# culiver/VAR

Hardware: AMD Instinct MI355X
Metric: 256x256 images/sec (CFG=1.5) VAR-d16 (higher is better)
Workload: dtype f32

## Files before the change

var_amd/csrc/winograd.hip:

```cpp
#include <cstdlib>
#include <type_traits>

#include "common.h"

namespace {

constexpr int WG_PT = 18;
constexpr int WG_NDMA = 21;
constexpr int WG_STAGE = WG_NDMA * 16 * 64;
constexpr int WG_ZSTR = 20;
constexpr int WG_LDS = 2 * WG_STAGE;
static_assert(8 * 64 * WG_ZSTR * 4 <= WG_LDS, "epilogue exchange must fit in the K-loop stages");

struct WinoP {
    const float* in; const float* u; const float* bias; const float* resid; float* out; double* gn_part;
    int H, W, Cin, Cout, ncg, pw, ppi;
};

__device__ __forceinline__ void wg_wait_dma_barrier() { asm volatile("s_waitcnt vmcnt(8)\n\ts_barrier" ::: "memory"); }

constexpr int WG_KO_NOEPI = 1, WG_KO_NOGN = 2, WG_KO_NORES = 4, WG_KO_NOBTDB = 8;

__device__ __forceinline__ int wg_swz(int pix) { return (pix >> 1) & 3; }

template <bool RES, bool GN, int KO>
__global__ void __launch_bounds__(256, 2) k_conv3x3_wino(WinoP p) {
    extern __shared__ __attribute__((aligned(16))) float smem[];
    const int tid = threadIdx.x, lane = tid & 63, wave = __builtin_amdgcn_readfirstlane(tid >> 6);
    const int r16 = lane & 15, kq = lane >> 4;
    int lin;
    {
        const int nwg = gridDim.x, bid = blockIdx.x, q = nwg >> 3, rem = nwg & 7, xcd = bid & 7, loc = bid >> 3;
        lin = (xcd < rem ? xcd * (q + 1) : rem * (q + 1) + (xcd - rem) * q) + loc;
    }
    const int cg = lin % p.ncg, pidx = lin / p.ncg, b = pidx / p.ppi, pi = pidx - b * p.ppi, py = pi / p.pw, px = pi - py * p.pw;
    const int y0 = py * 16, x0 = px * 16, c0 = cg * 32;
    const int H = p.H, W = p.W, Cin = p.Cin, Cout = p.Cout, nk = Cin >> 4;

    const int64_t img = (int64_t)H * W * Cin;
    const __amdgpu_buffer_rsrc_t rsrc = __builtin_amdgcn_make_buffer_rsrc((void*)(p.in + (int64_t)b * img), 0, (int)(img * 4), 0x00020000);
    uint32_t doff[6];
#pragma unroll
    for (int i = 0; i < 6; ++i) {
        const int pix = (wave + 4 * i) * 16 + (lane >> 2), c = lane & 3;
        const int yy = y0 - 1 + pix / WG_PT, xx = x0 - 1 + pix % WG_PT;
        const bool ok = pix < WG_PT * WG_PT && (unsigned)yy < (unsigned)H && (unsigned)xx < (unsigned)W;
        doff[i] = ok ? (uint32_t)((((int64_t)yy * W + xx) * Cin + ((c ^ wg_swz(pix)) << 2)) * 4) : 0x80000000u;
    }
    const uint32_t lds0 = (uint32_t)(uintptr_t)(__attribute__((address_space(3))) void*)smem;
    auto dma = [&](int kt, int st) {
#pragma unroll
        for (int i = 0; i < 6; ++i)
            if (wave + 4 * i < WG_NDMA) vh_dma16_buf(rsrc, doff[i], (uint32_t)kt * 64u, lds0 + st * WG_STAGE + (wave + 4 * i) * 1024);
    };

    const uint32_t ustr_xi = (uint32_t)nk * Cout * 64, ustr_kt = (uint32_t)Cout * 64;
    const __amdgpu_buffer_rsrc_t ursrc = __builtin_amdgcn_make_buffer_rsrc((void*)p.u, 0, (int)(16 * ustr_xi), 0x00020000);
    const uint32_t uoff = (uint32_t)((c0 + r16) * 16 + 4 * kq) * 4u;
    f32x4 u[4][2];
    auto load_u = [&](int kt, int j) {
#pragma unroll
        for (int cb = 0; cb < 2; ++cb)
            u[j][cb] = __builtin_bit_cast(f32x4, __builtin_amdgcn_raw_buffer_load_b128(
                ursrc, uoff, __builtin_amdgcn_readfirstlane((uint32_t)(4 * wave + j) * ustr_xi + (uint32_t)kt * ustr_kt + cb * 1024u), 0));
    };
    dma(0, 0);
#pragma unroll
    for (int j = 0; j < 4; ++j) { load_u(0, j); __builtin_amdgcn_sched_barrier(0); }

    const int ra = wave == 3 ? 1 : (wave == 2 ? 2 : wave), rb = wave == 0 ? 2 : (wave == 1 ? 2 : (wave == 2 ? 1 : 3));
    const float sg = wave == 1 ? 1.0f : -1.0f;
    uint32_t roff[2][4];
#pragma unroll
    for (int c = 0; c < 4; ++c) {
        const int pa = (2 * (r16 >> 3) + ra) * WG_PT + 2 * (r16 & 7) + c, pb = (2 * (r16 >> 3) + rb) * WG_PT + 2 * (r16 & 7) + c;
        roff[0][c] = (uint32_t)(pa * 64 + ((kq ^ wg_swz(pa)) << 4));
        roff[1][c] = (uint32_t)(pb * 64 + ((kq ^ wg_swz(pb)) << 4));
    }

    f32x4 acc[4][4][2];
#pragma unroll
    for (int j = 0; j < 4; ++j)
#pragma unroll
        for (int tb = 0; tb < 4; ++tb)
#pragma unroll
            for (int cb = 0; cb < 2; ++cb) acc[j][tb][cb] = f32x4{0.f, 0.f, 0.f, 0.f};

    const int et = tid & 63, eq = tid >> 6;
    const int ety = et >> 3, etx = et & 7;
    const int64_t obase = (((int64_t)b * H + y0 + 2 * ety) * W + x0 + 2 * etx) * Cout + c0 + 4 * eq;
    f32x4 b4[2], rs[2][2][2];
    auto epi_load = [&](int j) {
        if constexpr (KO & WG_KO_NOEPI) return;
        if (j == 0) { b4[0] = *(const f32x4*)(p.bias + c0 + 4 * eq); b4[1] = *(const f32x4*)(p.bias + c0 + 16 + 4 * eq); }
        if constexpr (RES) {
#pragma unroll
            for (int bb = 0; bb < 2; ++bb) rs[j >> 1][j & 1][bb] = *(const f32x4*)(p.resid + obase + ((int64_t)(j & 1) * W + bb) * Cout + (j >> 1) * 16);
        }
    };

    auto compute = [&](int st, int kt_dma, int kt_u, auto last) {
        const char* sb = (const char*)smem + st * WG_STAGE;
#pragma unroll
        for (int tb = 0; tb < 4; ++tb) {
            f32x4 da[4], db[4];
#pragma unroll
            for (int c = 0; c < 4; ++c) {
                da[c] = *(const f32x4*)(sb + roff[0][c] + tb * 72 * 64);
                db[c] = *(const f32x4*)(sb + roff[1][c] + tb * 72 * 64);
            }
            float e[4][4];
            if constexpr (!(KO & WG_KO_NOBTDB)) {
#pragma unroll
                for (int c = 0; c < 4; ++c)
#pragma unroll
                    for (int s = 0; s < 4; ++s) e[c][s] = __builtin_fmaf(sg, db[c][s], da[c][s]);
            }
#pragma unroll
            for (int j = 0; j < 4; ++j) {
#pragma unroll
                for (int s = 0; s < 4; ++s) {
                    float v;
                    if constexpr (KO & WG_KO_NOBTDB) v = (j & 1) ? db[j][s] : da[j][s];
                    else v = j == 0 ? e[0][s] - e[2][s] : (j == 1 ? e[1][s] + e[2][s] : (j == 2 ? e[2][s] - e[1][s] : e[1][s] - e[3][s]));
#pragma unroll
                    for (int cb = 0; cb < 2; ++cb) acc[j][tb][cb] = __builtin_amdgcn_mfma_f32_16x16x4f32(u[j][cb][s], v, acc[j][tb][cb], 0, 0, 0);
                }
                if (tb == 3) {
                    __builtin_amdgcn_sched_barrier(0);
                    if constexpr (decltype(last)::value) epi_load(j); else load_u(kt_u, j);
                }
            }
            __builtin_amdgcn_sched_barrier(0);
            if (tb == 0 && !decltype(last)::value) dma(kt_dma, st ^ 1);
        }
    };

    wg_wait_dma_barrier();
    int kt = 0;
    for (; kt + 2 < nk; kt += 2) {
        compute(0, kt + 1, kt + 1, std::false_type{});
        wg_wait_dma_barrier();
        compute(1, kt + 2, kt + 2, std::false_type{});
        wg_wait_dma_barrier();
    }
    compute(0, kt + 1, kt + 1, std::false_type{});
    wg_wait_dma_barrier();
    compute(1, 0, 0, std::true_type{});
    __builtin_amdgcn_s_barrier();
    if constexpr (KO & WG_KO_NOEPI) {
#pragma unroll
        for (int j = 0; j < 4; ++j)
#pragma unroll
            for (int tb = 0; tb < 4; ++tb)
#pragma unroll
                for (int cb = 0; cb < 2; ++cb) asm volatile("" :: "v"(acc[j][tb][cb]));
        return;
    }

    float* zb = smem;
    const int nblk = (H * W) >> 7;
#pragma unroll
    for (int cb = 0; cb < 2; ++cb) {
#pragma unroll
        for (int tb = 0; tb < 4; ++tb) {
            const f32x4 m0 = acc[0][tb][cb], m1 = acc[1][tb][cb], m2 = acc[2][tb][cb], m3 = acc[3][tb][cb];
            const f32x4 z0 = (m0 + m1) + m2, z1 = (m1 - m2) - m3;
            const int t = tb * 16 + r16;
            *(f32x4*)(zb + ((wave * 2 + 0) * 64 + t) * WG_ZSTR + 4 * kq) = z0;
            *(f32x4*)(zb + ((wave * 2 + 1) * 64 + t) * WG_ZSTR + 4 * kq) = z1;
        }
        __syncthreads();
        f32x4 z[4][2];
#pragma unroll
        for (int i = 0; i < 4; ++i)
#pragma unroll
            for (int bb = 0; bb < 2; ++bb) z[i][bb] = *(const f32x4*)(zb + ((i * 2 + bb) * 64 + et) * WG_ZSTR + 4 * eq);
        const int co = c0 + cb * 16 + 4 * eq;
        double gs[4] = {0.0, 0.0, 0.0, 0.0}, gq[4] = {0.0, 0.0, 0.0, 0.0};
#pragma unroll
        for (int a = 0; a < 2; ++a)
#pragma unroll
            for (int bb = 0; bb < 2; ++bb) {
                const f32x4 yv = a == 0 ? (z[0][bb] + z[1][bb]) + z[2][bb] : (z[1][bb] - z[2][bb]) - z[3][bb];
                f32x4 v = yv + b4[cb];
                const int64_t o = obase + ((int64_t)a * W + bb) * Cout + cb * 16;
                if constexpr (RES) v = rs[cb][a][bb] + v;
                *(f32x4*)(p.out + o) = v;
                if constexpr (GN) {
#pragma unroll
                    for (int e = 0; e < 4; ++e) { const double d = (double)v[e]; gs[e] += d; gq[e] += d * d; }
                }
            }
        if constexpr (GN) {
            const double t8[8] = {gs[0], gq[0], gs[1], gq[1], gs[2], gq[2], gs[3], gq[3]};
            const bool h4 = lane & 16, h3 = lane & 8, h2 = lane & 4;
            double r4[4], r2[2], r1;
#pragma unroll
            for (int i = 0; i < 4; ++i) r4[i] = (h4 ? t8[4 + i] : t8[i]) + __shfl_xor(h4 ? t8[i] : t8[4 + i], 16, 64);
#pragma unroll
            for (int i = 0; i < 2; ++i) r2[i] = (h3 ? r4[2 + i] : r4[i]) + __shfl_xor(h3 ? r4[i] : r4[2 + i], 8, 64);
            r1 = (h2 ? r2[1] : r2[0]) + __shfl_xor(h2 ? r2[0] : r2[1], 4, 64);
            r1 += __shfl_xor(r1, 2, 64);
            r1 += __shfl_xor(r1, 1, 64);
            if ((lane & 3) == 0)
                p.gn_part[(((int64_t)b * nblk + 2 * pi + (lane >> 5)) * Cout + co) * 2 + ((lane >> 2) & 7)] = r1;
        }
        if (cb == 0) __syncthreads();
    }
}

constexpr int WU_PS = 12;
constexpr int WU_NDMA = 8;
constexpr int WU_STAGE = WU_NDMA * 16 * 64;
constexpr int WU_LDS = 2 * WU_STAGE;

__device__ __forceinline__ void wu_wait_dma_barrier() { asm volatile("s_waitcnt vmcnt(9)\n\ts_barrier" ::: "memory"); }

template <bool GN>
__global__ void __launch_bounds__(256, 2) k_conv3x3_wino_up(WinoP p) {
    extern __shared__ __attribute__((aligned(16))) float smem[];
    const int tid = threadIdx.x, lane = tid & 63, wave = __builtin_amdgcn_readfirstlane(tid >> 6);
    const int r16 = lane & 15, kq = lane >> 4, th = wave & 1, ch = wave >> 1;
    int lin;
    {
        const int nwg = gridDim.x, bid = blockIdx.x, q = nwg >> 3, rem = nwg & 7, xcd = bid & 7, loc = bid >> 3;
        lin = (xcd < rem ? xcd * (q + 1) : rem * (q + 1) + (xcd - rem) * q) + loc;
    }
    const int cg = lin % p.ncg, pidx = lin / p.ncg, b = pidx / p.ppi, pi = pidx - b * p.ppi, py = pi / p.pw, px = pi - py * p.pw;
    const int y0 = py * 16, x0 = px * 16, c0 = cg * 32 + ch * 16;
    const int H = p.H, W = p.W, Hi = H >> 1, Wi = W >> 1, Cin = p.Cin, Cout = p.Cout, nk = Cin >> 4;

    const int64_t img = (int64_t)Hi * Wi * Cin;
    const __amdgpu_buffer_rsrc_t rsrc = __builtin_amdgcn_make_buffer_rsrc((void*)(p.in + (int64_t)b * img), 0, (int)(img * 4), 0x00020000);
    uint32_t doff[2];
#pragma unroll
    for (int i = 0; i < 2; ++i) {
        const int pix = (wave + 4 * i) * 16 + (lane >> 2), c = lane & 3;
        const int pr = pix / WU_PS, pc = pix - pr * WU_PS;
        const int yy = (y0 >> 1) - 1 + pr, xx = (x0 >> 1) - 1 + pc;
        const bool ok = pr < 10 && pc < 10 && (unsigned)yy < (unsigned)Hi && (unsigned)xx < (unsigned)Wi;
        doff[i] = ok ? (uint32_t)((((int64_t)yy * Wi + xx) * Cin + ((c ^ ((pr & 1) << 1)) << 2)) * 4) : 0x80000000u;
    }
    const uint32_t lds0 = (uint32_t)(uintptr_t)(__attribute__((address_space(3))) void*)smem;
    auto dma = [&](int kt, int st) __attribute__((always_inline)) {
#pragma unroll
        for (int i = 0; i < 2; ++i) vh_dma16_buf(rsrc, doff[i], (uint32_t)kt * 64u, lds0 + st * WU_STAGE + (wave + 4 * i) * 1024);
    };

    const __amdgpu_buffer_rsrc_t ursrc = __builtin_amdgcn_make_buffer_rsrc((void*)p.u, 0, (int)(64u * Cin * Cout), 0x00020000);
    const uint32_t uoff = (uint32_t)((c0 + r16) * 4 * Cin + 4 * kq) * 4u;
    f32x4 u[9];
    auto load_u = [&](int kt, int r) __attribute__((always_inline)) {
#pragma unroll
        for (int c = 0; c < 3; ++c)
            u[3 * r + c] = __builtin_bit_cast(f32x4, __builtin_amdgcn_raw_buffer_load_b128(
                ursrc, uoff, __builtin_amdgcn_readfirstlane((uint32_t)((((r == 2 ? 2 : 0) + (c == 2 ? 1 : 0)) * Cout * 4 + (r == 0 ? 0 : 2) + (c == 0 ? 0 : 1)) * Cin + 16 * kt) * 4u), 0));
    };
    dma(0, 0);
#pragma unroll
    for (int r = 0; r < 3; ++r) { load_u(0, r); __builtin_amdgcn_sched_barrier(0); }

    const int prow = 4 * th + (r16 >> 3), pbase = (prow * WU_PS + (r16 & 7)) * 64;
    const uint32_t roff_e = (uint32_t)(pbase + ((kq ^ ((prow & 1) << 1)) << 4)), roff_o = (uint32_t)(pbase + ((kq ^ (((prow + 1) & 1) << 1)) << 4));

    f32x4 acc[9][2];
#pragma unroll
    for (int j = 0; j < 9; ++j)
#pragma unroll
        for (int tb = 0; tb < 2; ++tb) acc[j][tb] = f32x4{0.f, 0.f, 0.f, 0.f};

    f32x4 b4;
    auto compute = [&](int st, int kt_dma, int kt_u, auto last) __attribute__((always_inline)) {
        const char* sb = (const char*)smem + st * WU_STAGE;
#pragma unroll
        for (int tb = 0; tb < 2; ++tb) {
            f32x4 d[3][3];
#pragma unroll
            for (int r = 0; r < 3; ++r)
#pragma unroll
                for (int c = 0; c < 3; ++c) d[r][c] = *(const f32x4*)(sb + (r == 1 ? roff_o : roff_e) + (r * WU_PS + c + tb * 2 * WU_PS) * 64);
#pragma unroll
            for (int r = 0; r < 3; ++r) {
                if (tb == 0) {
                    if (r == 0) u[1] = u[0] + u[1];
                    if (r == 1) { u[4] = u[1] + (u[3] + u[4]); u[3] = u[0] + u[3]; u[5] = u[2] + u[5]; }
                    if (r == 2) u[7] = u[6] + u[7];
                }
                f32x4 e[3];
#pragma unroll
                for (int c = 0; c < 3; ++c) e[c] = r == 0 ? d[0][c] - d[1][c] : (r == 1 ? d[1][c] : d[1][c] - d[2][c]);
                const f32x4 v[3] = {e[0] - e[1], e[1], e[1] - e[2]};
#pragma unroll
                for (int s = 0; s < 4; ++s)
#pragma unroll
                    for (int c = 0; c < 3; ++c) acc[3 * r + c][tb] = __builtin_amdgcn_mfma_f32_16x16x4f32(u[3 * r + c][s], v[c][s], acc[3 * r + c][tb], 0, 0, 0);
                if (tb == 1) {
                    __builtin_amdgcn_sched_barrier(0);
                    if constexpr (decltype(last)::value) { if (r == 0) b4 = *(const f32x4*)(p.bias + c0 + 4 * kq); } else load_u(kt_u, r);
                }
            }
            __builtin_amdgcn_sched_barrier(0);
            if (tb == 0 && !decltype(last)::value) dma(kt_dma, st ^ 1);
        }
    };
    wu_wait_dma_barrier();
    int kt = 0;
    for (; kt + 2 < nk; kt += 2) {
        compute(0, kt + 1, kt + 1, std::false_type{});
        wu_wait_dma_barrier();
        compute(1, kt + 2, kt + 2, std::false_type{});
        wu_wait_dma_barrier();
    }
    compute(0, kt + 1, kt + 1, std::false_type{});
    wu_wait_dma_barrier();
    compute(1, 0, 0, std::true_type{});

    const int nblk = (H * W) >> 7;
    double gs[4] = {0.0, 0.0, 0.0, 0.0}, gq[4] = {0.0, 0.0, 0.0, 0.0};
#pragma unroll
    for (int tb = 0; tb < 2; ++tb) {
        const int ty = 4 * th + 2 * tb + (r16 >> 3), tx = r16 & 7;
        const int64_t obase = (((int64_t)b * H + y0 + 2 * ty) * W + x0 + 2 * tx) * Cout + c0 + 4 * kq;
        f32x4 z[3][2];
#pragma unroll
        for (int r = 0; r < 3; ++r) {
            z[r][0] = acc[3 * r][tb] + acc[3 * r + 1][tb]; z[r][1] = acc[3 * r + 1][tb] - acc[3 * r + 2][tb];
        }
#pragma unroll
        for (int a = 0; a < 2; ++a)
#pragma unroll
            for (int bb = 0; bb < 2; ++bb) {
                const f32x4 v = (a == 0 ? z[0][bb] + z[1][bb] : z[1][bb] - z[2][bb]) + b4;
                *(f32x4*)(p.out + obase + ((int64_t)a * W + bb) * Cout) = v;
                if constexpr (GN) {
#pragma unroll
                    for (int e = 0; e < 4; ++e) { const double dd = (double)v[e]; gs[e] += dd; gq[e] += dd * dd; }
                }
            }
    }
    if constexpr (GN) {
        const double t8[8] = {gs[0], gq[0], gs[1], gq[1], gs[2], gq[2], gs[3], gq[3]};
        const bool h3 = lane & 8, h2 = lane & 4, h1 = lane & 2;
        double r4[4], r2[2], r1;
#pragma unroll
        for (int k = 0; k < 4; ++k) r4[k] = (h3 ? t8[4 + k] : t8[k]) + __shfl_xor(h3 ? t8[k] : t8[4 + k], 8, 64);
#pragma unroll
        for (int k = 0; k < 2; ++k) r2[k] = (h2 ? r4[2 + k] : r4[k]) + __shfl_xor(h2 ? r4[k] : r4[2 + k], 4, 64);
        r1 = (h1 ? r2[1] : r2[0]) + __shfl_xor(h1 ? r2[0] : r2[1], 2, 64);
        r1 += __shfl_xor(r1, 1, 64);
        if ((lane & 1) == 0)
            p.gn_part[(((int64_t)b * nblk + 2 * pi + th) * Cout + c0 + 4 * kq) * 2 + ((lane >> 1) & 7)] = r1;
    }
}

}

static bool wino_up_ok(const float* in, const float* w_phase, const float* bias, float* out, int B, int H, int W, int Cin, int Cout) {
    if (!in || !w_phase || !bias || !out || B <= 0 || H <= 0 || W <= 0 || Cin <= 0 || Cout <= 0) return false;
    if ((H & 15) || (W & 15) || (Cin & 31) || (Cout & 31)) return false;
    if ((((uintptr_t)in | (uintptr_t)w_phase | (uintptr_t)bias | (uintptr_t)out) & 15)) return false;
    if ((int64_t)(H / 2) * (W / 2) * Cin * 4 >= (1ll << 31) || 64ll * Cin * Cout >= (1ll << 31) || (int64_t)B * H * W >= (1ll << 31))
        return false;
    return (int64_t)B * (H / 16) * (W / 16) * (Cout / 32) < (1ll << 31);
}

extern "C" int varhip_conv3x3_wino_up_nhwc_f32(const float* in, const float* w_phase, const float* bias, float* out, double* gn_part,
                                               int B, int H, int W, int Cin, int Cout, varhip_stream_t stream) {
    if (!wino_up_ok(in, w_phase, bias, out, B, H, W, Cin, Cout)) return VARHIP_EINVAL;
    const int ppi = (H / 16) * (W / 16), ncg = Cout / 32;
    const int64_t nwg = (int64_t)B * ppi * ncg;
    WinoP p{};
    p.in = in; p.u = w_phase; p.bias = bias; p.resid = nullptr; p.out = out; p.gn_part = gn_part;
    p.H = H; p.W = W; p.Cin = Cin; p.Cout = Cout; p.ncg = ncg; p.pw = W / 16; p.ppi = ppi;
    const double npix = (double)B * H * W;
    VhScope scope(VH_FAM_CONV_WINO_UP, (hipStream_t)stream, 2.0 * (npix / 4.0) * 9.0 * Cin * Cout,
                  4.0 * (npix / 4.0 * Cin + npix * Cout + 16.0 * Cin * Cout));
    hipLaunchKernelGGL(gn_part ? k_conv3x3_wino_up<true> : k_conv3x3_wino_up<false>, dim3((unsigned)nwg), dim3(256), WU_LDS, (hipStream_t)stream, p);
    return vh_launch_status();
}

extern "C" { int vh_g_upconv_wino = 0; }
int vh_upconv_wino_try(const float* in, const float* w_phase, const float* bias, float* out, double* gn_part,
                       int B, int H, int W, int Cin, int Cout, hipStream_t stream) {
    if (!vh_g_upconv_wino || !wino_up_ok(in, w_phase, bias, out, B, H, W, Cin, Cout)) return 1;
    return varhip_conv3x3_wino_up_nhwc_f32(in, w_phase, bias, out, gn_part, B, H, W, Cin, Cout, (varhip_stream_t)stream);
}

extern "C" int varhip_conv3x3_wino_nhwc_f32(const float* in, const float* u, const float* bias, const float* resid, float* out, double* gn_part,
                                            int B, int H, int W, int Cin, int Cout, varhip_stream_t stream) {
    if (!in || !u || !bias || !out || B <= 0 || H <= 0 || W <= 0 || Cin <= 0 || Cout <= 0) return VARHIP_EINVAL;
    if ((H & 15) || (W & 15) || (Cin & 31) || (Cout & 31)) return VARHIP_EINVAL;
    if ((((uintptr_t)in | (uintptr_t)u | (uintptr_t)bias | (uintptr_t)out | (uintptr_t)resid) & 15)) return VARHIP_EINVAL;
    if ((int64_t)H * W * Cin * 4 >= (1ll << 31) || 64ll * Cin * Cout >= (1ll << 31) || (int64_t)B * H * W >= (1ll << 31))
        return VARHIP_EINVAL;
    const int ppi = (H / 16) * (W / 16), ncg = Cout / 32;
    const int64_t nwg = (int64_t)B * ppi * ncg;
    if (nwg >= (1ll << 31)) return VARHIP_EINVAL;
    WinoP p{};
    p.in = in; p.u = u; p.bias = bias; p.resid = resid; p.out = out; p.gn_part = gn_part;
    p.H = H; p.W = W; p.Cin = Cin; p.Cout = Cout; p.ncg = ncg; p.pw = W / 16; p.ppi = ppi;
    const double npix = (double)B * H * W;
    VhScope scope(VH_FAM_CONV_WINO, (hipStream_t)stream, 2.0 * (npix / 4.0) * 16.0 * Cin * Cout,
                  4.0 * (npix * Cin + npix * Cout * (resid ? 2.0 : 1.0) + 16.0 * Cin * Cout));
    static const int dbg = [] { const char* e = getenv("VARHIP_WINO_DBG"); return e ? atoi(e) : 0; }();
    const bool res = resid && !(dbg & WG_KO_NORES), gn = gn_part && !(dbg & WG_KO_NOGN);
    if ((dbg & WG_KO_NOBTDB) && !(res && gn)) return VARHIP_EINVAL;
    auto kfn = (dbg & WG_KO_NOEPI) ? k_conv3x3_wino<false, false, WG_KO_NOEPI> : (dbg & WG_KO_NOBTDB) ? k_conv3x3_wino<true, true, WG_KO_NOBTDB>
             : res ? (gn ? k_conv3x3_wino<true, true, 0> : k_conv3x3_wino<true, false, 0>)
                   : (gn ? k_conv3x3_wino<false, true, 0> : k_conv3x3_wino<false, false, 0>);
    hipLaunchKernelGGL(kfn, dim3((unsigned)nwg), dim3(256), WG_LDS, (hipStream_t)stream, p);
    return vh_launch_status();
}
```

var_amd/hip.py:

```python
import ctypes
import os

from . import abi

_HERE = os.path.dirname(os.path.abspath(__file__))
LIB_PATH = os.environ.get('VARHIP_LIB') or os.path.join(_HERE, 'libvar_hip.so')


class VarHipError(RuntimeError):
    pass


class _Lib:
    def __init__(self):
        if not os.path.exists(LIB_PATH):
            raise VarHipError(f'{LIB_PATH} not found: build it with `python -c "import __graft_entry__ as g; g.build()"` '
                              f'(or `make -C var_amd/csrc`). There is no CPU/PyTorch fallback for the sampling path.')
        self.so = ctypes.CDLL(LIB_PATH)
        self.fn = abi.bind(self.so, 'varhip_', with_stream=True)
        self.host = {name: getattr(self.so, 'varhip_' + name) for name in abi.SIGNATURES_HOST}

    def version(self) -> str:
        return self.fn['version']().decode()


_LIB = None


def lib() -> _Lib:
    global _LIB
    if _LIB is None:
        _LIB = _Lib()
    return _LIB


def _arg(a):
    if a is None:
        return None
    if hasattr(a, 'data_ptr'):
        return ctypes.c_void_p(a.data_ptr())
    return a


def current_stream() -> ctypes.c_void_p:
    import torch
    return ctypes.c_void_p(torch.cuda.current_stream().cuda_stream)


def call(name: str, *args, stream=None):
    L = lib()
    st = current_stream() if stream is None else stream
    rc = L.fn[name](*[_arg(a) for a in args], st)
    if rc != 0:
        raise VarHipError(f'varhip_{name} returned {rc}' + (' (VARHIP_EINVAL: unsupported shape/argument)' if rc == abi.EINVAL else ' (HIP launch error %d)' % (-rc - 1000)))


def call_host(name: str, *args):
    def arg(a):
        if hasattr(a, 'ctypes'):
            return ctypes.c_void_p(a.ctypes.data)
        return _arg(a)
    if name not in abi.SIGNATURES_HOST:
        raise VarHipError(f'varhip_{name} is not a host function')
    rc = lib().host[name](*[arg(a) for a in args])
    if rc != 0:
        raise VarHipError(f'varhip_{name} returned {rc}' + (' (VARHIP_EINVAL: unsupported shape/argument)' if rc == abi.EINVAL else ''))


def gn_scratch_elems(B, HW, C, G) -> int:
    return int(lib().fn['gn_scratch_elems'](B, HW, C, G))


def conv_gn_blocks(H, W, Cout, phase=False) -> int:
    return int(lib().fn['conv_gn_blocks'](H, W, Cout, 1 if phase else 0))


def upconv_winograd(on: bool):
    ctypes.c_int.in_dll(lib().so, 'vh_g_upconv_wino').value = 1 if on else 0


def conv16_gn_fusable(B, H, W, Cin, Cout) -> bool:
    return bool(lib().fn['conv16_gn_fusable'](B, H, W, Cin, Cout))


VQ_STATS_MAX_BLOCKS = abi.CONSTANTS['VQ_STATS_MAX_BLOCKS']


def vq_stats_blocks(n: int) -> int:
    return int(lib().so.varhip_vq_stats_blocks(n))


NFAM = abi.CONSTANTS['NFAM']


def timing_enable(on: bool, families=None):
    so = lib().so
    mask = -1
    if families is not None:
        names = [so.varhip_timing_name(i).decode() for i in range(NFAM)]
        mask = sum(1 << names.index(f) for f in families)
    so.varhip_timing_select(mask)
    so.varhip_timing_enable(1 if on else 0)


def timing_reset():
    lib().so.varhip_timing_reset()


def timing_read():
    n = abi_nfam = NFAM
    ms = (ctypes.c_double * n)(); fl = (ctypes.c_double * n)(); by = (ctypes.c_double * n)(); ln = (ctypes.c_int64 * n)()
    lib().so.varhip_timing_read(ms, fl, by, ln)
    return {lib().so.varhip_timing_name(i).decode(): dict(ms=ms[i], flops=fl[i], bytes=by[i], launches=int(ln[i])) for i in range(abi_nfam)}
```

Before: 158.1.

## Add wide 80-channel Winograd conv kernel tiling for Cout divisible by 80

Adds a second Winograd 3x3 conv kernel in which each workgroup covers 80 output channels over a half-height (8-row) patch, instead of 32 channels over a 16x16 patch. It is selected automatically when Cout is a multiple of 80, and it also admits Cout values that are not multiples of 32. The aim is to reuse each input tile across more output channels and to get a better grid fit for the VQ-VAE decoder conv shapes. The cost is more accumulator registers and a multi-pass epilogue through LDS, which may hurt occupancy.

New measurement: 159.8 (median of 6 runs). 1.01x the previous value.

```diff
diff --git a/var_amd/csrc/winograd.hip b/var_amd/csrc/winograd.hip
--- a/var_amd/csrc/winograd.hip
+++ b/var_amd/csrc/winograd.hip
@@ -207,6 +207,201 @@
                 p.gn_part[(((int64_t)b * nblk + 2 * pi + (lane >> 5)) * Cout + co) * 2 + ((lane >> 2) & 7)] = r1;
         }
         if (cb == 0) __syncthreads();
+    }
+}
+
+constexpr int WW_PH = 10;
+constexpr int WW_NDMA = 12;
+constexpr int WW_STAGE = WW_NDMA * 16 * 64;
+constexpr int WW_NCB = 5;
+constexpr int WW_ZBLK = 8 * 32 * WG_ZSTR;
+constexpr int WW_LDS = 2 * WW_ZBLK * 4;
+static_assert(2 * WW_STAGE <= WW_LDS, "the K-loop stages must fit in the epilogue exchange");
+
+__device__ __forceinline__ void ww_wait_dma_barrier() { asm volatile("s_waitcnt vmcnt(5)\n\ts_barrier" ::: "memory"); }
+
+template <bool RES, bool GN, int KO>
+__global__ void __launch_bounds__(256, 2) k_conv3x3_wino_wide(WinoP p) {
+    extern __shared__ __attribute__((aligned(16))) float smem[];
+    const int tid = threadIdx.x, lane = tid & 63, wave = __builtin_amdgcn_readfirstlane(tid >> 6);
+    const int r16 = lane & 15, kq = lane >> 4;
+    int lin;
+    {
+        const int nwg = gridDim.x, bid = blockIdx.x, q = nwg >> 3, rem = nwg & 7, xcd = bid & 7, loc = bid >> 3;
+        lin = (xcd < rem ? xcd * (q + 1) : rem * (q + 1) + (xcd - rem) * q) + loc;
+    }
+    const int cg = lin % p.ncg, hidx = lin / p.ncg, b = hidx / (2 * p.ppi), hp = hidx - b * 2 * p.ppi, pi = hp >> 1, hh = hp & 1;
+    const int py = pi / p.pw, px = pi - py * p.pw;
+    const int y0 = py * 16 + 8 * hh, x0 = px * 16, c0 = cg * 80;
+    const int H = p.H, W = p.W, Cin = p.Cin, Cout = p.Cout, nk = Cin >> 4;
+
+    const int64_t img = (int64_t)H * W * Cin;
+    const __amdgpu_buffer_rsrc_t rsrc = __builtin_amdgcn_make_buffer_rsrc((void*)(p.in + (int64_t)b * img), 0, (int)(img * 4), 0x00020000);
+    uint32_t doff[3];
+#pragma unroll
+    for (int i = 0; i < 3; ++i) {
+        const int pix = (wave + 4 * i) * 16 + (lane >> 2), c = lane & 3;
+        const int yy = y0 - 1 + pix / WG_PT, xx = x0 - 1 + pix % WG_PT;
+        const bool ok = pix < WW_PH * WG_PT && (unsigned)yy < (unsigned)H && (unsigned)xx < (unsigned)W;
+        doff[i] = ok ? (uint32_t)((((int64_t)yy * W + xx) * Cin + ((c ^ wg_swz(pix)) << 2)) * 4) : 0x80000000u;
+    }
+    const uint32_t lds0 = (uint32_t)(uintptr_t)(__attribute__((address_space(3))) void*)smem;
+    auto dma = [&](int kt, int st) __attribute__((always_inline)) {
+#pragma unroll
+        for (int i = 0; i < 3; ++i) vh_dma16_buf(rsrc, doff[i], (uint32_t)kt * 64u, lds0 + st * WW_STAGE + (wave + 4 * i) * 1024);
+    };
+
+    const uint32_t ustr_xi = (uint32_t)nk * Cout * 64, ustr_kt = (uint32_t)Cout * 64;
+    const __amdgpu_buffer_rsrc_t ursrc = __builtin_amdgcn_make_buffer_rsrc((void*)p.u, 0, (int)(16 * ustr_xi), 0x00020000);
+    const uint32_t uoff = (uint32_t)((c0 + r16) * 16 + 4 * kq) * 4u;
+    f32x4 u[WW_NCB];
+    auto load_u = [&](int kt, int j, int cb) __attribute__((always_inline)) {
+        u[cb] = __builtin_bit_cast(f32x4, __builtin_amdgcn_raw_buffer_load_b128(
+            ursrc, uoff, __builtin_amdgcn_readfirstlane((uint32_t)(4 * wave + j) * ustr_xi + (uint32_t)kt * ustr_kt + cb * 1024u), 0));
+    };
+    dma(0, 0);
+#pragma unroll
+    for (int cb = 0; cb < WW_NCB; ++cb) { load_u(0, 0, cb); __builtin_amdgcn_sched_barrier(0); }
+
+    const int ra = wave == 3 ? 1 : (wave == 2 ? 2 : wave), rb = wave == 0 ? 2 : (wave == 1 ? 2 : (wave == 2 ? 1 : 3));
+    const float sg = wave == 1 ? 1.0f : -1.0f;
+    uint32_t roff[2][4];
+#pragma unroll
+    for (int c = 0; c < 4; ++c) {
+        const int pa = (2 * (r16 >> 3) + ra) * WG_PT + 2 * (r16 & 7) + c, pb = (2 * (r16 >> 3) + rb) * WG_PT + 2 * (r16 & 7) + c;
+        roff[0][c] = (uint32_t)(pa * 64 + ((kq ^ wg_swz(pa)) << 4));
+        roff[1][c] = (uint32_t)(pb * 64 + ((kq ^ wg_swz(pb)) << 4));
+    }
+
+    f32x4 acc[4][2][WW_NCB];
+#pragma unroll
+    for (int j = 0; j < 4; ++j)
+#pragma unroll
+        for (int tb = 0; tb < 2; ++tb)
+#pragma unroll
+            for (int cb = 0; cb < WW_NCB; ++cb) acc[j][tb][cb] = f32x4{0.f, 0.f, 0.f, 0.f};
+
+    auto build_v = [&](const char* sb, int j, f32x4 (&v)[2]) __attribute__((always_inline)) {
+        const int ca = j == 0 ? 0 : (j == 2 ? 2 : 1), cc = j == 0 ? 2 : (j == 1 ? 2 : (j == 2 ? 1 : 3));
+#pragma unroll
+        for (int tb = 0; tb < 2; ++tb) {
+            const f32x4 daa = *(const f32x4*)(sb + roff[0][ca] + tb * 72 * 64), dba = *(const f32x4*)(sb + roff[1][ca] + tb * 72 * 64);
+            const f32x4 dac = *(const f32x4*)(sb + roff[0][cc] + tb * 72 * 64), dbc = *(const f32x4*)(sb + roff[1][cc] + tb * 72 * 64);
+            if constexpr (KO & WG_KO_NOBTDB) {
+                asm volatile("" :: "v"(dba), "v"(dbc));
+#pragma unroll
+                for (int s = 0; s < 4; ++s) v[tb][s] = (s & 1) ? dac[s] : daa[s];
+            } else {
+#pragma unroll
+                for (int s = 0; s < 4; ++s) {
+                    const float ea = __builtin_fmaf(sg, dba[s], daa[s]), ec = __builtin_fmaf(sg, dbc[s], dac[s]);
+                    v[tb][s] = j == 1 ? ea + ec : ea - ec;
+                }
+            }
+        }
+    };
+
+    auto compute = [&](int st, int kt, int kt_n, auto last) __attribute__((always_inline)) {
+        const char* sb = (const char*)smem + st * WW_STAGE;
+        f32x4 v[2], vn[2];
+        build_v(sb, 0, v);
+#pragma unroll
+        for (int j = 0; j < 4; ++j) {
+#pragma unroll
+            for (int cb = 0; cb < WW_NCB; ++cb) {
+#pragma unroll
+                for (int s = 0; s < 4; ++s)
+#pragma unroll
+                    for (int tb = 0; tb < 2; ++tb) acc[j][tb][cb] = __builtin_amdgcn_mfma_f32_16x16x4f32(u[cb][s], v[tb][s], acc[j][tb][cb], 0, 0, 0);
+                __builtin_amdgcn_sched_barrier(0);
+                if (j < 3) load_u(kt, j + 1, cb);
+                else if constexpr (!decltype(last)::value) load_u(kt_n, 0, cb);
+                if (cb == 1 && j < 3) build_v(sb, j + 1, vn);
+                __builtin_amdgcn_sched_barrier(0);
+            }
+            if (j == 0 && !decltype(last)::value) dma(kt_n, st ^ 1);
+            if (j < 3) { v[0] = vn[0]; v[1] = vn[1]; }
+        }
+    };
+
+    ww_wait_dma_barrier();
+    int kt = 0;
+    for (; kt + 2 < nk; kt += 2) {
+        compute(0, kt, kt + 1, std::false_type{});
+        ww_wait_dma_barrier();
+        compute(1, kt + 1, kt + 2, std::false_type{});
+        ww_wait_dma_barrier();
+    }
+    compute(0, kt, kt + 1, std::false_type{});
+    ww_wait_dma_barrier();
+    compute(1, kt + 1, 0, std::true_type{});
+    __builtin_amdgcn_s_barrier();
+
+    float* zb = smem;
+    const int nblk = (H * W) >> 7;
+    const int et = lane & 31, sel = lane >> 5, eq = wave, ety = et >> 3, etx = et & 7;
+    const int64_t obase = (((int64_t)b * H + y0 + 2 * ety) * W + x0 + 2 * etx) * Cout + c0 + 4 * eq;
+#pragma unroll
+    for (int ps = 0; ps < 3; ++ps) {
+        const bool active = 2 * ps + sel < WW_NCB;
+        const int cbe = active ? 2 * ps + sel : WW_NCB - 1, zsel = active ? sel : 0;
+        const f32x4 b4 = *(const f32x4*)(p.bias + c0 + 16 * cbe + 4 * eq);
+        f32x4 rs[2][2];
+        if constexpr (RES) {
+#pragma unroll
+            for (int a = 0; a < 2; ++a)
+#pragma unroll
+                for (int bb = 0; bb < 2; ++bb) rs[a][bb] = *(const f32x4*)(p.resid + obase + ((int64_t)a * W + bb) * Cout + cbe * 16);
+        }
+#pragma unroll
+        for (int c2 = 0; c2 < 2; ++c2) {
+            const int cb = 2 * ps + c2;
+            if (cb >= WW_NCB) continue;
+#pragma unroll
+            for (int tb = 0; tb < 2; ++tb) {
+                const f32x4 m0 = acc[0][tb][cb], m1 = acc[1][tb][cb], m2 = acc[2][tb][cb], m3 = acc[3][tb][cb];
+                const f32x4 z0 = (m0 + m1) + m2, z1 = (m1 - m2) - m3;
+                const int t = tb * 16 + r16;
+                *(f32x4*)(zb + c2 * WW_ZBLK + ((wave * 2 + 0) * 32 + t) * WG_ZSTR + 4 * kq) = z0;
+                *(f32x4*)(zb + c2 * WW_ZBLK + ((wave * 2 + 1) * 32 + t) * WG_ZSTR + 4 * kq) = z1;
+            }
+        }
+        __syncthreads();
+        f32x4 z[4][2];
+#pragma unroll
+        for (int i = 0; i < 4; ++i)
+#pragma unroll
+            for (int bb = 0; bb < 2; ++bb) z[i][bb] = *(const f32x4*)(zb + zsel * WW_ZBLK + ((i * 2 + bb) * 32 + et) * WG_ZSTR + 4 * eq);
+        const int co = c0 + cbe * 16 + 4 * eq;
+        double gs[4] = {0.0, 0.0, 0.0, 0.0}, gq[4] = {0.0, 0.0, 0.0, 0.0};
+#pragma unroll
+        for (int a = 0; a < 2; ++a)
+#pragma unroll
+            for (int bb = 0; bb < 2; ++bb) {
+                const f32x4 yv = a == 0 ? (z[0][bb] + z[1][bb]) + z[2][bb] : (z[1][bb] - z[2][bb]) - z[3][bb];
+                f32x4 v = yv + b4;
+                if constexpr (RES) v = rs[a][bb] + v;
+                if (active) *(f32x4*)(p.out + obase + ((int64_t)a * W + bb) * Cout + cbe * 16) = v;
+                if constexpr (GN) {
+#pragma unroll
+                    for (int e = 0; e < 4; ++e) { const double d = (double)v[e]; gs[e] += d; gq[e] += d * d; }
+                }
+            }
+        if constexpr (GN) {
+            const double t8[8] = {gs[0], gq[0], gs[1], gq[1], gs[2], gq[2], gs[3], gq[3]};
+            const bool h4 = lane & 16, h3 = lane & 8, h2 = lane & 4;
+            double r4[4], r2[2], r1;
+#pragma unroll
+            for (int i = 0; i < 4; ++i) r4[i] = (h4 ? t8[4 + i] : t8[i]) + __shfl_xor(h4 ? t8[i] : t8[4 + i], 16, 64);
+#pragma unroll
+            for (int i = 0; i < 2; ++i) r2[i] = (h3 ? r4[2 + i] : r4[i]) + __shfl_xor(h3 ? r4[i] : r4[2 + i], 8, 64);
+            r1 = (h2 ? r2[1] : r2[0]) + __shfl_xor(h2 ? r2[0] : r2[1], 4, 64);
+            r1 += __shfl_xor(r1, 2, 64);
+            r1 += __shfl_xor(r1, 1, 64);
+            if (active && (lane & 3) == 0)
+                p.gn_part[(((int64_t)b * nblk + 2 * pi + hh) * Cout + co) * 2 + ((lane >> 2) & 7)] = r1;
+        }
+        if (ps < 2) __syncthreads();
     }
 }
 
@@ -387,16 +582,32 @@
     return varhip_conv3x3_wino_up_nhwc_f32(in, w_phase, bias, out, gn_part, B, H, W, Cin, Cout, (varhip_stream_t)stream);
 }
 
+static int vh_g_wino_force_shape = [] { const char* e = getenv("VARHIP_WINO_SHAPE"); const int t = e ? atoi(e) : -1; return (t == 0 || t == 1) ? t : -1; }();
+static int vh_g_wino_last_shape = -1;
+extern "C" int varhip_wino_force_shape(int shape) { vh_g_wino_force_shape = (shape == 0 || shape == 1) ? shape : -1; return 0; }
+extern "C" int varhip_wino_last_shape(void) { return vh_g_wino_last_shape; }
+extern "C" int varhip_wino_auto_shape(int H, int W, int Cin, int Cout) {
+    (void)H; (void)W; (void)Cin;
+    return Cout > 0 && Cout % 80 == 0;
+}
+extern "C" int varhip_wino_pick_shape(int H, int W, int Cin, int Cout) {
+    if (Cout <= 0 || Cout % 80) return 0;
+    if (Cout & 31) return 1;
+    return vh_g_wino_force_shape >= 0 ? vh_g_wino_force_shape : varhip_wino_auto_shape(H, W, Cin, Cout);
+}
+
 extern "C" int varhip_conv3x3_wino_nhwc_f32(const float* in, const float* u, const float* bias, const float* resid, float* out, double* gn_part,
                                             int B, int H, int W, int Cin, int Cout, varhip_stream_t stream) {
     if (!in || !u || !bias || !out || B <= 0 || H <= 0 || W <= 0 || Cin <= 0 || Cout <= 0) return VARHIP_EINVAL;
-    if ((H & 15) || (W & 15) || (Cin & 31) || (Cout & 31)) return VARHIP_EINVAL;
+    if ((H & 15) || (W & 15) || (Cin & 31) || ((Cout & 31) && (Cout % 80))) return VARHIP_EINVAL;
     if ((((uintptr_t)in | (uintptr_t)u | (uintptr_t)bias | (uintptr_t)out | (uintptr_t)resid) & 15)) return VARHIP_EINVAL;
     if ((int64_t)H * W * Cin * 4 >= (1ll << 31) || 64ll * Cin * Cout >= (1ll << 31) || (int64_t)B * H * W >= (1ll << 31))
         return VARHIP_EINVAL;
-    const int ppi = (H / 16) * (W / 16), ncg = Cout / 32;
-    const int64_t nwg = (int64_t)B * ppi * ncg;
+    const int shape = varhip_wino_pick_shape(H, W, Cin, Cout);
+    const int ppi = (H / 16) * (W / 16), ncg = shape ? Cout / 80 : Cout / 32;
+    const int64_t nwg = (int64_t)B * ppi * ncg * (shape ? 2 : 1);
     if (nwg >= (1ll << 31)) return VARHIP_EINVAL;
+    vh_g_wino_last_shape = shape;
     WinoP p{};
     p.in = in; p.u = u; p.bias = bias; p.resid = resid; p.out = out; p.gn_part = gn_part;
     p.H = H; p.W = W; p.Cin = Cin; p.Cout = Cout; p.ncg = ncg; p.pw = W / 16; p.ppi = ppi;
@@ -406,6 +617,14 @@
     static const int dbg = [] { const char* e = getenv("VARHIP_WINO_DBG"); return e ? atoi(e) : 0; }();
     const bool res = resid && !(dbg & WG_KO_NORES), gn = gn_part && !(dbg & WG_KO_NOGN);
     if ((dbg & WG_KO_NOBTDB) && !(res && gn)) return VARHIP_EINVAL;
+    if (shape) {
+        if (dbg & ~WG_KO_NOBTDB) return VARHIP_EINVAL;
+        auto wfn = (dbg & WG_KO_NOBTDB) ? k_conv3x3_wino_wide<true, true, WG_KO_NOBTDB>
+                 : res ? (gn ? k_conv3x3_wino_wide<true, true, 0> : k_conv3x3_wino_wide<true, false, 0>)
+                       : (gn ? k_conv3x3_wino_wide<false, true, 0> : k_conv3x3_wino_wide<false, false, 0>);
+        hipLaunchKernelGGL(wfn, dim3((unsigned)nwg), dim3(256), WW_LDS, (hipStream_t)stream, p);
+        return vh_launch_status();
+    }
     auto kfn = (dbg & WG_KO_NOEPI) ? k_conv3x3_wino<false, false, WG_KO_NOEPI> : (dbg & WG_KO_NOBTDB) ? k_conv3x3_wino<true, true, WG_KO_NOBTDB>
              : res ? (gn ? k_conv3x3_wino<true, true, 0> : k_conv3x3_wino<true, false, 0>)
                    : (gn ? k_conv3x3_wino<false, true, 0> : k_conv3x3_wino<false, false, 0>);
diff --git a/var_amd/hip.py b/var_amd/hip.py
--- a/var_amd/hip.py
+++ b/var_amd/hip.py
@@ -79,6 +79,24 @@
     ctypes.c_int.in_dll(lib().so, 'vh_g_upconv_wino').value = 1 if on else 0
 
 
+def _wino_hook(name, nargs):
+    fn = getattr(lib().so, 'varhip_wino_' + name)
+    fn.argtypes, fn.restype = [ctypes.c_int] * nargs, ctypes.c_int
+    return fn
+
+
+def wino_force_shape(shape: int):
+    _wino_hook('force_shape', 1)(int(shape))
+
+
+def wino_last_shape() -> int:
+    return int(_wino_hook('last_shape', 0)())
+
+
+def wino_auto_shape(H, W, Cin, Cout) -> int:
+    return int(_wino_hook('auto_shape', 4)(H, W, Cin, Cout))
+
+
 def conv16_gn_fusable(B, H, W, Cin, Cout) -> bool:
     return bool(lib().fn['conv16_gn_fusable'](B, H, W, Cin, Cout))
 
```
